# wenxiaoshuai/Points-Matching

Hardware: AMD Instinct MI355X
Metric: descriptor-pair distances/s (BF-L2 2-NN + ratio stage); RANSAC hypotheses/s in `ransac` (higher is better)
Workload: dtype f32

## Files before the change

points_matching_amd/csrc/knn_coarse_kernels.hpp:

```cpp
#pragma once
#include <type_traits>

#include "knn_shared.hpp"

namespace pm_knn {
namespace {

template <bool NO_EPI, bool NO_STAGE, bool NO_BARRIER, bool NO_LDSREAD>
struct Abl {
    static constexpr bool no_epi = NO_EPI;
    static constexpr bool no_stage = NO_STAGE;
    static constexpr bool no_barrier = NO_BARRIER;
    static constexpr bool no_ldsread = NO_LDSREAD;
    static __device__ __forceinline__ void stamp(int) {}
};
typedef Abl<false, false, false, false> AblNone;

struct WgTile { int qb, split; };
__device__ __forceinline__ WgTile wg_tile(bool tiled)
{
    const int nx = gridDim.x, ny = gridDim.y;
    if (!tiled || (nx & 3) || (ny & 1)) return WgTile{static_cast<int>(blockIdx.x), static_cast<int>(blockIdx.y)};
    const int L = blockIdx.y * nx + blockIdx.x;
    const int x = L & 7, j = L >> 3;
    const int tw = nx >> 2, th = ny >> 1;
    return WgTile{(x & 3) * tw + j % tw, (x >> 2) * th + j / tw};
}

template <typename ABL>
__device__ __forceinline__ void tile_barrier()
{
    if constexpr (ABL::no_barrier) asm volatile("" ::: "memory");
    else __syncthreads();
}

__device__ __forceinline__ float embed_lid(float w, unsigned keep_mask, unsigned lid)
{
    return __uint_as_float((__float_as_uint(w) & keep_mask) | (lid & ~keep_mask));
}

__device__ __forceinline__ void top4_insert(f32x4& c, float x)
{
    const float n0 = fmaxf(x, c[0]);
    const float n1 = __builtin_amdgcn_fmed3f(x, c[0], c[1]);
    const float n2 = __builtin_amdgcn_fmed3f(x, c[1], c[2]);
    const float n3 = __builtin_amdgcn_fmed3f(x, c[2], c[3]);
    c[0] = n0; c[1] = n1; c[2] = n2; c[3] = n3;
}

__device__ __forceinline__ void merge_halves(f32x4& cl, int h)
{
    f32x4 own, other;
#pragma unroll
    for (int i = 0; i < 4; ++i) {
        own[i] = __uint_as_float(__float_as_uint(cl[i]) | static_cast<unsigned>(h));
        other[i] = __shfl_xor(own[i], 32, 64);
    }
    cl = own;
#pragma unroll
    for (int i = 0; i < 4; ++i) top4_insert(cl, other[i]);
}

__device__ __forceinline__ float group_max(const f32x16& acc, int g)
{
    return fmaxf(fmaxf(fmaxf(acc[4 * g], acc[4 * g + 1]), acc[4 * g + 2]), acc[4 * g + 3]);
}

template <int NCH, bool FULL, int TT>
struct KnnTile {
    static constexpr int DP = NCH * 8;
    static constexpr int LDT = DP + 4;
    static constexpr int F4_PER_ROW = DP / 4;
    static constexpr int NSTG = TT * F4_PER_ROW / 256;
    static_assert(TT * F4_PER_ROW % 256 == 0, "tile must split evenly over the workgroup");

    f32x4 stg[NSTG];
    float stg_n;

    __device__ __forceinline__ void load(const float* __restrict__ T, const float* __restrict__ tnorm, int tile,
                                         int nt, int dim, int tid)
    {
#pragma unroll
        for (int i = 0; i < NSTG; ++i) {
            const int f = tid + 256 * i;
            const int row = f / F4_PER_ROW, c4 = f % F4_PER_ROW;
            int g = tile * TT + row;
            g = g < nt ? g : nt - 1;
            int col = 4 * c4;
            if (!FULL) col = col < dim ? col : dim - 4;
            f32x4 v = *reinterpret_cast<const f32x4*>(T + static_cast<size_t>(g) * dim + col);
            if (!FULL && 4 * c4 >= dim) v = f32x4{0.f, 0.f, 0.f, 0.f};
            stg[i] = v;
        }
        const int gn = tile * TT + (tid & (TT - 1));
        const float nrm = tnorm[gn < nt ? gn : nt - 1];
        stg_n = gn < nt ? -0.5f * nrm : -0.5f * KNN_BIG;
    }
    __device__ __forceinline__ void store(float* __restrict__ Ts, int buf, int tid) const
    {
#pragma unroll
        for (int i = 0; i < NSTG; ++i) {
            const int f = tid + 256 * i;
            const int row = f / F4_PER_ROW, c4 = f % F4_PER_ROW;
            *reinterpret_cast<f32x4*>(Ts + (buf * TT + row) * LDT + 4 * c4) = stg[i];
        }
        if (tid < TT) *reinterpret_cast<f32x4*>(Ts + (buf * TT + tid) * LDT + DP) = f32x4{stg_n, 0.f, 0.f, 0.f};
    }
};

template <int NCH, bool FULL, int NB, bool EPI, typename ABL>
__device__ __forceinline__ void knn_tile_compute(float* __restrict__ Ts, int buf, int r, int h,
                                                 const f32x4 (&qf)[NCH], f32x16 (&a)[NB], const f32x16 (&p)[NB],
                                                 unsigned pbase, unsigned keep_mask, f32x4& cl,
                                                 KnnTile<NCH, FULL, NB * 32>& st, const float* __restrict__ T,
                                                 const float* __restrict__ tnorm, int next_tile, int nt, int dim,
                                                 int tid)
{
    constexpr int DP = NCH * 8;
    constexpr int LDT = DP + 4;
    constexpr int TT = NB * 32;
    static_assert(NCH >= 4, "the in-chain schedule needs at least 4 chunks");
    const float* tb = Ts + buf * TT * LDT + r * LDT + 4 * h;
    const float one_or_zero = h == 0 ? 1.f : 0.f;
    float sda[NB];
    f32x4 xn[NB];
#pragma unroll
    for (int blk = 0; blk < NB; ++blk) {
        sda[blk] = Ts[buf * TT * LDT + (32 * blk + r) * LDT + DP + h];
        xn[blk] = *reinterpret_cast<const f32x4*>(tb + 32 * blk * LDT);
    }
    {
        const f32x16 zero = {0.f, 0.f, 0.f, 0.f, 0.f, 0.f, 0.f, 0.f, 0.f, 0.f, 0.f, 0.f, 0.f, 0.f, 0.f, 0.f};
#pragma unroll
        for (int blk = 0; blk < NB; ++blk)
            a[blk] = __builtin_amdgcn_mfma_f32_32x32x2f32(sda[blk], one_or_zero, zero, 0, 0, 0);
    }
#pragma unroll
    for (int c = 0; c < NCH; ++c) {
        f32x4 x[NB];
#pragma unroll
        for (int blk = 0; blk < NB; ++blk) x[blk] = xn[blk];
        if constexpr (!ABL::no_ldsread) {
            if (c + 1 < NCH) {
#pragma unroll
                for (int blk = 0; blk < NB; ++blk)
                    xn[blk] = *reinterpret_cast<const f32x4*>(tb + 32 * blk * LDT + 8 * (c + 1));
            }
        }
#pragma unroll
        for (int t = 0; t < 4; ++t)
#pragma unroll
            for (int blk = 0; blk < NB; ++blk)
                a[blk] = __builtin_amdgcn_mfma_f32_32x32x2f32(x[blk][t], qf[c][t], a[blk], 0, 0, 0);
        if constexpr (!ABL::no_stage) {
            if (c == 0) st.load(T, tnorm, next_tile, nt, dim, tid);
            if (c == NCH - 2) st.store(Ts, buf ^ 1, tid);
        }
        if (EPI && !ABL::no_epi) {
            constexpr int NG = 4 * NB;
#pragma unroll
            for (int g = (c == 0 ? 0 : (c - 1) * NG / (NCH - 1)); g < (c == 0 ? 0 : c * NG / (NCH - 1)); ++g)
                top4_insert(cl, embed_lid(group_max(p[g >> 2], g & 3), keep_mask, (pbase + static_cast<unsigned>(g)) << 1));
            asm volatile("" : "+v"(cl[0]), "+v"(cl[1]), "+v"(cl[2]), "+v"(cl[3]));
        }
    }
}

template <int NB>
__device__ __forceinline__ void knn_select_all(const f32x16 (&p)[NB], unsigned pbase, unsigned keep_mask, f32x4& cl)
{
#pragma unroll
    for (int g = 0; g < 4 * NB; ++g)
        top4_insert(cl, embed_lid(group_max(p[g >> 2], g & 3), keep_mask, (pbase + static_cast<unsigned>(g)) << 1));
}

template <int NCH, bool FULL, int TT, typename ABL>
__global__ __launch_bounds__(256, (TT == 64 ? 2 : 1)) void knn_l2_mfma(
    const float* __restrict__ Q, const float* __restrict__ T, const float* __restrict__ tnorm, int nq,
    int nt, int dim, int tiles_per_split, unsigned keep_mask, float* __restrict__ cand_val, int slots,
    const unsigned long long* __restrict__ stats, unsigned epoch, int only_if_ineligible)
{
    if (only_if_ineligible & 1) {
        const unsigned long long s1 = stats[1], s3 = stats[3];
        if (!(static_cast<unsigned>(s1 >> 32) == epoch && (s1 & 2ull) && static_cast<unsigned>(s3 >> 32) == epoch)) return;
    }
    using Tile = KnnTile<NCH, FULL, TT>;
    constexpr int LDT = Tile::LDT;
    constexpr int NB = TT / 32;
    constexpr unsigned IDS = 4 * NB;
    extern __shared__ __attribute__((aligned(16))) float smem[];
    float* Ts = smem;

    const int tid = threadIdx.x;
    const int lane = tid & 63, wave = tid >> 6;
    const int r = lane & 31, h = lane >> 5;
    const WgTile wg = wg_tile((only_if_ineligible & 2) != 0);
    const int qrow = wg.qb * QB + wave * 32 + r;
    const int qld = qrow < nq ? qrow : nq - 1;

    f32x4 qf[NCH];
#pragma unroll
    for (int c = 0; c < NCH; ++c) {
        const int k0 = 8 * c + 4 * h;
        int col = k0;
        if (!FULL) col = col < dim ? col : dim - 4;
        f32x4 v = *reinterpret_cast<const f32x4*>(Q + static_cast<size_t>(qld) * dim + col);
        if (!FULL && k0 >= dim) v = f32x4{0.f, 0.f, 0.f, 0.f};
        qf[c] = v;
    }

    const int ntiles = (nt + TT - 1) / TT;
    const int tile0 = wg.split * tiles_per_split;
    int tile1 = tile0 + tiles_per_split;
    if (tile1 > ntiles) tile1 = ntiles;

    f32x4 cl = {-KNN_BIG, -KNN_BIG, -KNN_BIG, -KNN_BIG};
    if (tile0 < tile1) {
        Tile st;
        st.load(T, tnorm, tile0, nt, dim, tid);
        st.store(Ts, 0, tid);
        __syncthreads();

        f32x16 accA[NB], accB[NB];
        int tix = 0;
        const int ntl = tile1 - tile0;
        knn_tile_compute<NCH, FULL, NB, false, ABL>(Ts, 0, r, h, qf, accA, accA, 0u, keep_mask, cl, st, T, tnorm,
                                               tile0 + 1, nt, dim, tid);
        tile_barrier<ABL>();
        ++tix;
        for (;;) {
            if (tix >= ntl) { knn_select_all<NB>(accA, static_cast<unsigned>(tix - 1) * IDS, keep_mask, cl); break; }
            knn_tile_compute<NCH, FULL, NB, true, ABL>(Ts, tix & 1, r, h, qf, accB, accA, static_cast<unsigned>(tix - 1) * IDS,
                                                  keep_mask, cl, st, T, tnorm, tile0 + tix + 1, nt, dim, tid);
            tile_barrier<ABL>();
            ++tix;
            if (tix >= ntl) { knn_select_all<NB>(accB, static_cast<unsigned>(tix - 1) * IDS, keep_mask, cl); break; }
            knn_tile_compute<NCH, FULL, NB, true, ABL>(Ts, tix & 1, r, h, qf, accA, accB, static_cast<unsigned>(tix - 1) * IDS,
                                                  keep_mask, cl, st, T, tnorm, tile0 + tix + 1, nt, dim, tid);
            tile_barrier<ABL>();
            ++tix;
        }
    }

    merge_halves(cl, h);
    if (qrow < nq && h == 0) {
        const size_t o = static_cast<size_t>(qrow) * slots + wg.split * KNN_C;
        *reinterpret_cast<f32x4*>(cand_val + o) = cl;
    }
}

template <int DP>
struct RouteF16T {
    static constexpr int NCH = DP / 16 + 1;
    static constexpr int ROW16 = (DP + 16) / 8;
    static constexpr int LDS_ROW16 = ROW16 + 1;
    static_assert(LDS_ROW16 % 2 == 1 && (H_TT * LDS_ROW16) % 64 == 0, "conflict-free rows, whole DMA pieces");
    static constexpr int GPB = 4;
    static constexpr bool MERGE = true;
    static constexpr bool SEEDED = false;
    typedef f16x8 frag;
    typedef f32x16 acc;
    typedef f32x4 list;
    static __device__ __forceinline__ acc zero()
    {
        return acc{0.f, 0.f, 0.f, 0.f, 0.f, 0.f, 0.f, 0.f, 0.f, 0.f, 0.f, 0.f, 0.f, 0.f, 0.f, 0.f};
    }
    static __device__ __forceinline__ acc mfma(frag a, frag b, acc c)
    {
        return __builtin_amdgcn_mfma_f32_32x32x16_f16(a, b, c, 0, 0, 0);
    }
    static __device__ __forceinline__ list empty() { return list{-KNN_BIG, -KNN_BIG, -KNN_BIG, -KNN_BIG}; }
    static __device__ __forceinline__ void select(const acc& a, unsigned par, unsigned gid, list& cl, int g)
    {
        top4_insert(cl, embed_lid(group_max(a, g), par, gid));
    }
    static __device__ __forceinline__ void merge(list& cl, int h) { merge_halves(cl, h); }
    static __device__ __forceinline__ void put(list& cl, float x) { top4_insert(cl, x); }
};
typedef RouteF16T<128> RouteF16;
static_assert(RouteF16::NCH == H_NCH && RouteF16::ROW16 == H_ROW16 && RouteF16::LDS_ROW16 == H_LDS_ROW16, "knn_shared.hpp constants");

template <int BITS>
struct RouteI8T {
    static_assert(BITS == 256 || BITS == 512, "descriptor bits padded to 256 or 512");
    static constexpr int NCH = BITS / 32;
    static constexpr int ROW16 = BITS / 16;
    static constexpr int LDS_ROW16 = ROW16 + 1;
    static_assert(LDS_ROW16 % 2 == 1 && (H_TT * LDS_ROW16) % 64 == 0, "conflict-free rows, whole DMA pieces");
    static constexpr int GPB = 2;
    static constexpr bool MERGE = false;
    static constexpr bool SEEDED = false;
    typedef i32x4 frag;
    typedef i32x16 acc;
    typedef i32x4 list;
    static __device__ __forceinline__ acc zero() { return acc{0, 0, 0, 0, 0, 0, 0, 0, 0, 0, 0, 0, 0, 0, 0, 0}; }
    static __device__ __forceinline__ acc mfma(frag a, frag b, acc c)
    {
        return __builtin_amdgcn_mfma_i32_32x32x32_i8(a, b, c, 0, 0, 0);
    }
    static __device__ __forceinline__ list empty() { return list{I8_EMPTY, I8_EMPTY, I8_EMPTY, I8_EMPTY}; }
    static __device__ __forceinline__ int med3(int a, int b, int c) { return max(min(a, b), min(max(a, b), c)); }
    static __device__ __forceinline__ void select(const acc& a, unsigned par, unsigned gid, list& cl, int g)
    {
        const int m0 = max(max(a[8 * g], a[8 * g + 1]), a[8 * g + 2]);
        const int m1 = max(max(a[8 * g + 3], a[8 * g + 4]), a[8 * g + 5]);
        const int m = max(max(max(m0, m1), a[8 * g + 6]), a[8 * g + 7]);
        const int x = static_cast<int>((static_cast<unsigned>(m) << I8_SHIFT) | gid);
        (void)par;
        insert(cl, x);
    }
    static __device__ __forceinline__ void put(list& cl, int x) { insert(cl, x); }
    static __device__ __forceinline__ void insert(list& cl, int x)
    {
        const int n0 = max(x, cl[0]);
        const int n1 = med3(x, cl[0], cl[1]);
        const int n2 = med3(x, cl[1], cl[2]);
        const int n3 = med3(x, cl[2], cl[3]);
        cl[0] = n0; cl[1] = n1; cl[2] = n2; cl[3] = n3;
    }
    static __device__ __forceinline__ void merge(list& cl, int h)
    {
#pragma unroll
        for (int i = 0; i < 4; ++i) cl[i] = cl[i] == I8_EMPTY ? I8_EMPTY : (cl[i] | h);
    }
};
struct RouteI8 : RouteI8T<I8_BITS> {};
static_assert(RouteI8::NCH == I8_NCH && RouteI8::ROW16 == I8_ROW16 && RouteI8::LDS_ROW16 == I8_LDS_ROW16, "knn_shared.hpp constants");
typedef RouteI8T<I8W_BITS> RouteI8W;
static_assert(RouteI8W::NCH == I8W_NCH && RouteI8W::ROW16 == I8W_ROW16 && RouteI8W::LDS_ROW16 == 33, "knn_shared.hpp constants");
static_assert(sizeof(uint4) * 2 * H_TT * RouteI8W::LDS_ROW16 == 135168, "two 512-bit tile buffers: one workgroup per CU");

struct RouteF16S : RouteF16 {
    static constexpr int NCH = F16S_NCH;
    static constexpr int ROW16 = F16S_ROW16;
    static constexpr int LDS_ROW16 = F16S_LDS_ROW16;
    static constexpr bool SEEDED = true;
};

template <int GPB_>
struct RouteU8T {
    static constexpr int NCH = U8_NCH;
    static constexpr int ROW16 = U8_ROW16;
    static constexpr int LDS_ROW16 = U8_LDS_ROW16;
    static constexpr int GPB = GPB_;
    static constexpr int GROUP = 16 / GPB_;
    static constexpr bool MERGE = true;
    static constexpr bool SEEDED = true;
    typedef i32x4 frag;
    typedef i32x16 acc;
    typedef i32x4 list;
    static __device__ __forceinline__ acc zero() { return acc{0, 0, 0, 0, 0, 0, 0, 0, 0, 0, 0, 0, 0, 0, 0, 0}; }
    static __device__ __forceinline__ acc mfma(frag a, frag b, acc c)
    {
        return __builtin_amdgcn_mfma_i32_32x32x32_i8(a, b, c, 0, 0, 0);
    }
    static __device__ __forceinline__ list empty() { return list{I8_EMPTY, I8_EMPTY, I8_EMPTY, I8_EMPTY}; }
    static __device__ __forceinline__ int max3(int a, int b, int c) { return max(max(a, b), c); }
    static __device__ __forceinline__ void select(const acc& a, unsigned par, unsigned gid, list& cl, int g)
    {
        int m;
        if constexpr (GROUP == 4) {
            m = max(max3(a[4 * g], a[4 * g + 1], a[4 * g + 2]), a[4 * g + 3]);
        } else if constexpr (GROUP == 8) {
            const int m0 = max3(a[8 * g], a[8 * g + 1], a[8 * g + 2]);
            const int m1 = max3(m0, a[8 * g + 3], a[8 * g + 4]);
            m = max(max3(m1, a[8 * g + 5], a[8 * g + 6]), a[8 * g + 7]);
        } else {
            const int m0 = max3(a[0], a[1], a[2]), m1 = max3(a[3], a[4], a[5]), m2 = max3(a[6], a[7], a[8]);
            const int m3 = max3(a[9], a[10], a[11]), m4 = max3(a[12], a[13], a[14]);
            m = max(max3(m0, m1, m2), max3(m3, m4, a[15]));
        }
        (void)par;
        RouteI8::insert(cl, static_cast<int>((static_cast<unsigned>(m) << U8_SHIFT) | gid));
    }
    static __device__ __forceinline__ void put(list& cl, int x) { RouteI8::insert(cl, x); }
    static __device__ __forceinline__ void merge(list& cl, int h)
    {
        list own, other;
#pragma unroll
        for (int i = 0; i < 4; ++i) {
            own[i] = cl[i] == I8_EMPTY ? I8_EMPTY : (cl[i] | h);
            other[i] = __shfl_xor(own[i], 32, 64);
        }
        cl = own;
#pragma unroll
        for (int i = 0; i < 4; ++i) RouteI8::insert(cl, other[i]);
    }
};
typedef RouteU8T<4> RouteU8;

template <typename R, int THREADS>
struct HTile {
    static constexpr int TOTAL = H_TT * R::ROW16;
    static constexpr int PIECES = (TOTAL + THREADS - 1) / THREADS;
    static constexpr bool EVEN = TOTAL % THREADS == 0;
    uint4 stg[PIECES];
    __device__ __forceinline__ void load(const uint4* __restrict__ Th, int tile, int tid)
    {
#pragma unroll
        for (int i = 0; i < PIECES; ++i) {
            int f = tid + THREADS * i;
            if (!EVEN) f = f < TOTAL ? f : TOTAL - 1;
            stg[i] = Th[static_cast<size_t>(tile) * TOTAL + f];
        }
    }
    __device__ __forceinline__ void store(uint4* __restrict__ hsm, int buf, int tid) const
    {
#pragma unroll
        for (int i = 0; i < PIECES; ++i) {
            const int f = tid + THREADS * i;
            const int row = f / R::ROW16, c8 = f % R::ROW16;
            if (EVEN || f < TOTAL) hsm[(buf * H_TT + row) * R::LDS_ROW16 + c8] = stg[i];
        }
    }
};

template <typename R, int THREADS>
struct HTileDma {
    static constexpr int NW = THREADS / 64;
    static constexpr int SLOTS = H_TT * R::LDS_ROW16;
    static_assert(SLOTS % 64 == 0, "the padded tile must be a whole number of 1-KiB pieces");
    static constexpr int NPIECES = SLOTS / 64;
    static constexpr int PER_WAVE = (NPIECES + NW - 1) / NW;
    static constexpr int TOTAL = H_TT * R::ROW16;
    unsigned src[PER_WAVE];
    __device__ __forceinline__ void init(int lane, int wave)
    {
#pragma unroll
        for (int i = 0; i < PER_WAVE; ++i) {
            const int p = wave + NW * i;
            const int s = 64 * (p < NPIECES ? p : NPIECES - 1) + lane;
            const int row = s / R::LDS_ROW16, c = s % R::LDS_ROW16;
            src[i] = static_cast<unsigned>(row * R::ROW16 + (c < R::ROW16 ? c : R::ROW16 - 1));
        }
    }
    __device__ __forceinline__ void issue(__amdgpu_buffer_rsrc_t rsrc, int tile, uint4* __restrict__ hsm, int buf, int wave) const
    {
        typedef __attribute__((address_space(3))) void* lptr_t;
        const int soff = tile * (TOTAL * 16);
#pragma unroll
        for (int i = 0; i < PER_WAVE; ++i) {
            const int p = wave + NW * i;
            if (p < NPIECES) {
                uint4* l = hsm + buf * SLOTS + 64 * p;
                __builtin_amdgcn_raw_ptr_buffer_load_lds(rsrc, (lptr_t)l, 16, static_cast<int>(src[i]) * 16, soff, 0, 0);
            }
        }
    }
};

struct Seed64 { uint4 v[4]; };
template <typename R, int NQB, bool EPI, typename ABL>
__device__ __forceinline__ void h_block(const uint4* __restrict__ tb, const uint4* __restrict__ sb,
                                        const typename R::frag (&qf)[NQB][R::NCH],
                                        typename R::acc (&a)[NQB], const typename R::acc (&p)[NQB], unsigned pbase,
                                        unsigned par, typename R::list (&cl)[NQB])
{
    typedef typename R::frag frag;
    typename R::acc seed = R::zero();
    if constexpr (R::SEEDED) seed = __builtin_bit_cast(typename R::acc, Seed64{{sb[0], sb[1], sb[2], sb[3]}});
    frag ring[3];
#pragma unroll
    for (int c = 0; c < 3; ++c) ring[c] = *reinterpret_cast<const frag*>(tb + 2 * c);
#pragma unroll
    for (int c = 0; c < R::NCH; ++c) {
        const frag x = ring[c % 3];
        if constexpr (!ABL::no_ldsread) {
            if (c + 3 < R::NCH) ring[c % 3] = *reinterpret_cast<const frag*>(tb + 2 * (c + 3));
        }
#pragma unroll
        for (int qb = 0; qb < NQB; ++qb) a[qb] = R::mfma(x, qf[qb][c], c == 0 ? seed : a[qb]);
        if constexpr (ABL::no_epi) {
            if (EPI && c == 1) {
#pragma unroll
                for (int qb = 0; qb < NQB; ++qb)
#pragma unroll
                    for (int e = 0; e < 16; ++e) asm volatile("" ::"v"(p[qb][e]));
            }
        }
        if (EPI && c >= 1 && !ABL::no_epi) {
            constexpr int NGB = R::GPB * NQB;
#pragma unroll
            for (int e = (c - 1) * NGB / (R::NCH - 1); e < c * NGB / (R::NCH - 1); ++e)
                R::select(p[e % NQB], par, (pbase + static_cast<unsigned>(e / NQB)) << 1, cl[e % NQB], e / NQB);
            if (NQB == 2)
                asm volatile("" : "+v"(cl[0][0]), "+v"(cl[0][1]), "+v"(cl[0][2]), "+v"(cl[0][3]), "+v"(cl[NQB - 1][0]),
                             "+v"(cl[NQB - 1][1]), "+v"(cl[NQB - 1][2]), "+v"(cl[NQB - 1][3]));
            else
                asm volatile("" : "+v"(cl[0][0]), "+v"(cl[0][1]), "+v"(cl[0][2]), "+v"(cl[0][3]));
        }
    }
}

template <typename R, int NQB, bool FIRST, typename ABL>
__device__ __forceinline__ void h_tile(const uint4* __restrict__ tb, const uint4* __restrict__ sb,
                                       const typename R::frag (&qf)[NQB][R::NCH], typename R::acc (&A)[NQB],
                                       typename R::acc (&B)[NQB], unsigned lb, unsigned par, typename R::list (&cl)[NQB])
{
    typedef typename R::frag frag;
    typedef typename R::acc acc;
    constexpr int NCH = R::NCH, STEPS = 4 * NCH, PF = 3;
    constexpr unsigned G = R::GPB;
    auto a_ptr = [&](int step) { return reinterpret_cast<const frag*>(tb + (step / NCH) * 32 * R::LDS_ROW16 + 2 * (step % NCH)); };
    auto seed_of = [&](int blk) {
        if constexpr (R::SEEDED) {
            const uint4* p = sb + 8 * blk;
            return __builtin_bit_cast(acc, Seed64{{p[0], p[1], p[2], p[3]}});
        } else {
            return R::zero();
        }
    };
    frag ring[PF];
#pragma unroll
    for (int i = 0; i < PF; ++i) ring[i] = *a_ptr(i);
    acc seed = seed_of(0);
#pragma unroll
    for (int s_ = 0; s_ < STEPS; ++s_) {
        const int blk = s_ / NCH, c = s_ % NCH;
        const frag x = ring[s_ % PF];
        if constexpr (!ABL::no_ldsread) {
            if (s_ + PF < STEPS) ring[s_ % PF] = *a_ptr(s_ + PF);
        }
        acc(&cur)[NQB] = (blk & 1) ? B : A;
        const acc(&prev)[NQB] = (blk & 1) ? A : B;
#pragma unroll
        for (int qb = 0; qb < NQB; ++qb) cur[qb] = R::mfma(x, qf[qb][c], c == 0 ? seed : cur[qb]);
        if (c == 0 && blk < 3) seed = seed_of(blk + 1);
        const bool epi = !(FIRST && blk == 0);
        if constexpr (ABL::no_epi) {
            if (epi && c == 1) {
#pragma unroll
                for (int qb = 0; qb < NQB; ++qb)
#pragma unroll
                    for (int e = 0; e < 16; ++e) asm volatile("" ::"v"(prev[qb][e]));
            }
        }
        if (epi && c >= 1 && !ABL::no_epi) {
            constexpr int NGB = R::GPB * NQB;
            const unsigned pbase = lb + G * static_cast<unsigned>(blk) - G;
#pragma unroll
            for (int e = (c - 1) * NGB / (NCH - 1); e < c * NGB / (NCH - 1); ++e)
                R::select(prev[e % NQB], par, (pbase + static_cast<unsigned>(e / NQB)) << 1, cl[e % NQB], e / NQB);
            if (NQB == 2)
                asm volatile("" : "+v"(cl[0][0]), "+v"(cl[0][1]), "+v"(cl[0][2]), "+v"(cl[0][3]), "+v"(cl[NQB - 1][0]),
                             "+v"(cl[NQB - 1][1]), "+v"(cl[NQB - 1][2]), "+v"(cl[NQB - 1][3]));
            else
                asm volatile("" : "+v"(cl[0][0]), "+v"(cl[0][1]), "+v"(cl[0][2]), "+v"(cl[0][3]));
        }
    }
}

template <typename R, int NQB, bool DMA, int GR, int S, typename ABL>
__global__ __launch_bounds__(H_QB / (32 * NQB) * 64 * GR, (R::NCH > 9 ? (NQB == 2 ? 1 : 2) : (NQB == 2 ? 2 : 4))) void knn_mfma_rows288(
    const uint4* __restrict__ Qh, const uint4* __restrict__ Th, const uint4* __restrict__ seeds_g, int nq, int nt,
    int tiles_per_split, unsigned par, typename R::list* __restrict__ cand_val, int slots,
    const unsigned long long* __restrict__ stats, unsigned epoch, int mode)
{
    static_assert(S == 1 || ((S == 2 || S == 4) && GR == 1 && DMA && R::SEEDED), "super-tiles: the seeded LDS-DMA form, one row group");
    ABL::stamp(0);
    typedef typename R::frag frag;
    typedef typename R::acc acc;
    typedef typename R::list list;
    constexpr int WPG = H_QB / (32 * NQB);
    constexpr int THREADS = WPG * 64 * GR;
    static_assert(GR == 1 || (GR == 2 && NQB == 2 && R::MERGE), "row groups: the 64-query form of a merged-list route");
    if (mode & 1) {
        const unsigned long long s1 = stats[1], s3 = stats[3];
        if (static_cast<unsigned>(s1 >> 32) == epoch && (s1 & 2ull) && static_cast<unsigned>(s3 >> 32) == epoch)
            return;
    }
    extern __shared__ __attribute__((aligned(16))) uint4 hsm[];
    static_assert(!R::SEEDED || DMA, "the seeded routes stage by LDS-DMA only");
    constexpr int TILE_SLOTS = H_TT * R::LDS_ROW16;
    uint4* const ssm = hsm + 2 * S * TILE_SLOTS;
    const int tid = threadIdx.x, lane = tid & 63, wave = tid >> 6;
    const int r = lane & 31, h = lane >> 5;
    const int gw = wave % WPG, grp = wave / WPG;
    const WgTile wg = wg_tile((mode & 2) != 0);
    const int qbase = wg.qb * H_QB + gw * 32 * NQB;

    HTile<R, THREADS> st;
    HTileDma<R, THREADS> dma;
    const int ntiles = (nt + H_TT - 1) / H_TT;
    const int tile0 = wg.split * tiles_per_split;
    const __amdgpu_buffer_rsrc_t t_rsrc = __builtin_amdgcn_make_buffer_rsrc(
        const_cast<uint4*>(Th), 0, ntiles * (H_TT * R::ROW16 * 16), 0x00020000);
    const __amdgpu_buffer_rsrc_t s_rsrc = __builtin_amdgcn_make_buffer_rsrc(
        const_cast<uint4*>(R::SEEDED ? seeds_g : Th), 0, (ntiles + 1) * SEED_TILE_BYTES, 0x00020000);
    auto seed_issue = [&](int tile, int buf, int i) {
        typedef __attribute__((address_space(3))) void* lptr_t;
        if (R::SEEDED && wave == THREADS / 64 - 1 - i)
            __builtin_amdgcn_raw_ptr_buffer_load_lds(s_rsrc, (lptr_t)(ssm + 64 * buf), 16, lane * 16, tile * SEED_TILE_BYTES, 0, 0);
    };
    int tile1 = tile0 + tiles_per_split;
    if (tile1 > ntiles) tile1 = ntiles;
    const int ntl = tile1 - tile0;
    static_assert(S <= THREADS / 64, "one wave per seed piece of a super-tile");
    auto super_issue = [&](int u, int b) {
#pragma unroll
        for (int i = 0; i < S; ++i) {
            if constexpr (S == 1) {
                const int t = tile0 + u < ntiles ? tile0 + u : (tile0 + u - 1 < ntiles ? tile0 + u - 1 : ntiles - 1);
                dma.issue(t_rsrc, t, hsm, b, wave);
                seed_issue(t, b, 0);
            } else if (S * u + i < ntl) {
                dma.issue(t_rsrc, tile0 + S * u + i, hsm, b * S + i, wave);
                seed_issue(tile0 + S * u + i, b * S + i, i);
            }
        }
    };
    ABL::stamp(18);
    if (DMA) {
        dma.init(lane, wave);
        super_issue(0, 0);
        ABL::stamp(19);
    } else {
        st.load(Th, tile0 < ntiles ? tile0 : ntiles - 1, tid);
    }
    frag qf[NQB][R::NCH];
#pragma unroll
    for (int qb = 0; qb < NQB; ++qb)
#pragma unroll
        for (int c = 0; c < R::NCH; ++c) {
            if constexpr (R::SEEDED && R::NCH == U8_NCH)
                qf[qb][c] = *reinterpret_cast<const frag*>(Qh + (static_cast<size_t>((qbase >> 5) + qb) * R::NCH + c) * 64 + lane);
            else
                qf[qb][c] = *reinterpret_cast<const frag*>(Qh + static_cast<size_t>(qbase + 32 * qb + r) * R::ROW16 + 2 * c + h);
        }
    ABL::stamp(1);
#pragma unroll
    for (int qb = 0; qb < NQB; ++qb)
#pragma unroll
        for (int c = 0; c < R::NCH; ++c) {
            typedef unsigned u32x4 __attribute__((ext_vector_type(4)));
            u32x4 t = __builtin_bit_cast(u32x4, qf[qb][c]);
            asm volatile("" : "+v"(t));
            qf[qb][c] = __builtin_bit_cast(frag, t);
        }

    list cl[NQB];
#pragma unroll
    for (int qb = 0; qb < NQB; ++qb) cl[qb] = R::empty();

    if (tile0 < tile1) {
        if (!DMA) st.store(hsm, 0, tid);
        __syncthreads();
        ABL::stamp(2);
        acc A[NQB], B[NQB];
        for (int u = 0; u < (ntl + S - 1) / S; ++u) {
            const int buf = u & 1;
            constexpr unsigned G = R::GPB;
            if constexpr (!ABL::no_stage) {
                if (DMA) super_issue(u + 1, buf ^ 1);
                else st.load(Th, tile0 + u + 1 < ntiles ? tile0 + u + 1 : tile0 + u, tid);
            }
            if constexpr (GR == 1) {
#pragma unroll
                for (int i = 0; i < S; ++i) {
                    const int tix = S * u + i;
                    if (S > 1 && tix >= ntl) break;
                    const uint4* tb = hsm + ((buf * S + i) * H_TT + r) * R::LDS_ROW16 + h;
                    const uint4* sb = ssm + 64 * (buf * S + i) + 4 * h;
                    const unsigned lb = static_cast<unsigned>(tix) * (4u * G);
                    if (tix == 0) h_block<R, NQB, false, ABL>(tb, sb, qf, A, A, 0u, par, cl);
                    else h_block<R, NQB, true, ABL>(tb, sb, qf, A, B, lb - G, par, cl);
                    h_block<R, NQB, true, ABL>(tb + 32 * R::LDS_ROW16, sb + 8, qf, B, A, lb, par, cl);
                    h_block<R, NQB, true, ABL>(tb + 64 * R::LDS_ROW16, sb + 16, qf, A, B, lb + G, par, cl);
                    if constexpr (!ABL::no_stage) {
                        if (!DMA) st.store(hsm, buf ^ 1, tid);
                    }
                    h_block<R, NQB, true, ABL>(tb + 96 * R::LDS_ROW16, sb + 24, qf, B, A, lb + 2u * G, par, cl);
                }
            } else {
                const int tix = u;
                const uint4* tb = hsm + (buf * H_TT + r) * R::LDS_ROW16 + h;
                const uint4* sb = ssm + 64 * buf + 4 * h;
                const unsigned lb = static_cast<unsigned>(tix) * (4u * G);
                const uint4* tg = tb + grp * 64 * R::LDS_ROW16;
                const uint4* sg = sb + 16 * grp;
                const unsigned gb = lb + 2u * static_cast<unsigned>(grp) * G;
                if (tix == 0) h_block<R, NQB, false, ABL>(tg, sg, qf, A, A, 0u, par, cl);
                else h_block<R, NQB, true, ABL>(tg, sg, qf, A, B, gb - 3u * G, par, cl);
                if constexpr (!ABL::no_stage) {
                    if (!DMA) st.store(hsm, buf ^ 1, tid);
                }
                h_block<R, NQB, true, ABL>(tg + 32 * R::LDS_ROW16, sg + 8, qf, B, A, gb, par, cl);
            }
            tile_barrier<ABL>();
            if (u < 13) ABL::stamp(3 + u);
        }
        const unsigned lb = static_cast<unsigned>(tile1 - tile0 - 1) * (4u * R::GPB) +
                            (GR == 1 ? 3u : 2u * static_cast<unsigned>(grp) + 1u) * R::GPB;
#pragma unroll
        for (int qb = 0; qb < NQB; ++qb)
#pragma unroll
            for (int g = 0; g < R::GPB; ++g) R::select(B[qb], par, (lb + static_cast<unsigned>(g)) << 1, cl[qb], g);
    }
    ABL::stamp(16);
    if constexpr (GR == 2) {
        list* xs = reinterpret_cast<list*>(hsm);
#pragma unroll
        for (int qb = 0; qb < NQB; ++qb) {
            R::merge(cl[qb], h);
            if (grp == 1) xs[(gw * NQB + qb) * 64 + lane] = cl[qb];
        }
        __syncthreads();
        if (grp == 1) return;
#pragma unroll
        for (int qb = 0; qb < NQB; ++qb) {
            const list o = xs[(gw * NQB + qb) * 64 + lane];
#pragma unroll
            for (int i = 0; i < 4; ++i) R::put(cl[qb], o[i]);
            const int q = qbase + 32 * qb + r;
            if (q < nq && h == 0) cand_val[(static_cast<size_t>(q) * slots + wg.split * KNN_C) / KNN_C] = cl[qb];
        }
        return;
    }
#pragma unroll
    for (int qb = 0; qb < NQB; ++qb) {
        const int q = qbase + 32 * qb + r;
        R::merge(cl[qb], h);
        if (R::MERGE) {
            if (q < nq && h == 0) cand_val[(static_cast<size_t>(q) * slots + wg.split * KNN_C) / KNN_C] = cl[qb];
        } else {
            if (q < nq) cand_val[(static_cast<size_t>(q) * slots + (wg.split * 2 + h) * KNN_C) / KNN_C] = cl[qb];
        }
    }
    ABL::stamp(17);
}

template <int N>
__device__ __forceinline__ void wait_vmcnt_imm() { asm volatile("s_waitcnt vmcnt(%0)" ::"n"(N) : "memory"); }
template <int BASE>
__device__ __forceinline__ void wait_tiles(int ahead, bool plus)
{
    static_assert(7 * (BASE + 1) <= 63, "vmcnt is a 6-bit counter");
#define PM_W(A_) case A_: if (plus) wait_vmcnt_imm<A_ * (BASE + 1)>(); else wait_vmcnt_imm<A_ * BASE>(); break;
    switch (ahead) {
        PM_W(1) PM_W(2) PM_W(3) PM_W(4) PM_W(5) PM_W(6) PM_W(7)
        default: wait_vmcnt_imm<0>(); break;
    }
#undef PM_W
}

template <typename FRAG>
__device__ __forceinline__ FRAG untracked_load16(const void* p)
{
    typedef unsigned u32x4 __attribute__((ext_vector_type(4)));
    u32x4 v;
    asm volatile("global_load_dwordx4 %0, %1, off" : "=&v"(v) : "v"(p) : "memory");
    return __builtin_bit_cast(FRAG, v);
}
template <typename FRAG>
__device__ __forceinline__ void pin_after_wait(FRAG& f)
{
    typedef unsigned u32x4 __attribute__((ext_vector_type(4)));
    u32x4 t = __builtin_bit_cast(u32x4, f);
    asm volatile("" : "+v"(t)::"memory");
    f = __builtin_bit_cast(FRAG, t);
}

template <typename R, int NQB, int WAVES, int NBUF, bool SPLIT, typename ABL>
__global__ __launch_bounds__(WAVES * 64, WAVES / 4) void knn_mfma_ring(
    const uint4* __restrict__ Qh, const uint4* __restrict__ Th, const uint4* __restrict__ seeds_g, int nq, int nt,
    int tiles_per_split, unsigned par, typename R::list* __restrict__ cand_val, int slots, int mode, int pro)
{
    typedef typename R::frag frag;
    typedef typename R::acc acc;
    typedef typename R::list list;
    constexpr int THREADS = WAVES * 64;
    constexpr int QB_WG = WAVES * 32 * NQB;
    constexpr int TILE_SLOTS = H_TT * R::LDS_ROW16;
    typedef HTileDma<R, THREADS> Dma;
    static_assert(NBUF >= 3 && NBUF <= 8, "ring of three to eight buffers (wait_tiles covers up to 7 tiles in flight)");
    extern __shared__ __attribute__((aligned(16))) uint4 hsm[];
    uint4* const ssm = hsm + NBUF * TILE_SLOTS;
    int* const arrive = reinterpret_cast<int*>(ssm + NBUF * 64);
    int* const done = arrive + NBUF;
    const int tid = threadIdx.x, lane = tid & 63, wave = tid >> 6;
    const int r = lane & 31, h = lane >> 5;
    const WgTile wg = wg_tile((mode & 2) != 0);
    const int qbase = wg.qb * QB_WG + wave * 32 * NQB;
    ABL::stamp(0);
    if constexpr (SPLIT) {
        if (tid < 2 * NBUF) arrive[tid] = 0;
        asm volatile("s_waitcnt lgkmcnt(0)" ::: "memory");
        __builtin_amdgcn_s_barrier();
        asm volatile("" ::: "memory");
    }
    auto poll = [&](int* ctr, int target) {
        for (;;) {
            const int v = __builtin_amdgcn_readfirstlane(__hip_atomic_load(ctr, __ATOMIC_RELAXED, __HIP_MEMORY_SCOPE_WORKGROUP));
            if (v >= target) break;
            __builtin_amdgcn_s_sleep(1);
        }
        asm volatile("" ::: "memory");
    };
    auto bump = [&](int* ctr) {
        if (lane == 0) __hip_atomic_fetch_add(ctr, 1, __ATOMIC_RELAXED, __HIP_MEMORY_SCOPE_WORKGROUP);
    };

    const int ntiles = (nt + H_TT - 1) / H_TT;
    const int tile0 = wg.split * tiles_per_split;
    int tile1 = tile0 + tiles_per_split;
    if (tile1 > ntiles) tile1 = ntiles;
    const int ntl = tile1 - tile0;

    frag qf[NQB][R::NCH];
#pragma unroll
    for (int qb = 0; qb < NQB; ++qb)
#pragma unroll
        for (int c = 0; c < R::NCH; ++c)
            qf[qb][c] = untracked_load16<frag>(Qh + static_cast<size_t>(qbase + 32 * qb + r) * R::ROW16 + 2 * c + h);

    const __amdgpu_buffer_rsrc_t t_rsrc = __builtin_amdgcn_make_buffer_rsrc(
        const_cast<uint4*>(Th), 0, ntiles * (H_TT * R::ROW16 * 16), 0x00020000);
    const __amdgpu_buffer_rsrc_t s_rsrc = __builtin_amdgcn_make_buffer_rsrc(
        const_cast<uint4*>(R::SEEDED ? seeds_g : Th), 0, (ntiles + 1) * SEED_TILE_BYTES, 0x00020000);
    Dma dma;
    dma.init(lane, wave);
    constexpr int BASE = Dma::NPIECES / Dma::NW;
    const int own = (Dma::NPIECES - wave + Dma::NW - 1) / Dma::NW + ((R::SEEDED && wave == Dma::NW - 1) ? 1 : 0);
    const bool plus = __builtin_amdgcn_readfirstlane(own) != BASE;
    static_assert(Dma::NPIECES >= Dma::NW, "every wave issues at least one piece");
    auto request = [&](int t) {
        typedef __attribute__((address_space(3))) void* lptr_t;
        const int buf = t % NBUF;
        dma.issue(t_rsrc, tile0 + t, hsm, buf, wave);
        if (R::SEEDED && wave == Dma::NW - 1)
            __builtin_amdgcn_raw_ptr_buffer_load_lds(s_rsrc, (lptr_t)(ssm + 64 * buf), 16, lane * 16, (tile0 + t) * SEED_TILE_BYTES, 0, 0);
    };
    int next = 0;
    auto pump = [&](int done_below, int most) {
        for (int n = 0; n < most && next < ntl && next < done_below + NBUF; ++n) {
            if constexpr (SPLIT) {
                if (next >= NBUF) poll(&done[next % NBUF], WAVES * (next / NBUF));
            }
            request(next);
            ++next;
        }
    };
    pump(0, pro);
    if constexpr (SPLIT) {
        if (ntl > 0) {
            asm volatile("s_waitcnt vmcnt(0)" ::: "memory");
            bump(&arrive[0]);
        }
    }
    ABL::stamp(1);

    list cl[NQB];
#pragma unroll
    for (int qb = 0; qb < NQB; ++qb) cl[qb] = R::empty();

    if (ntl > 0) {
        acc A[NQB], B[NQB];
        constexpr unsigned G = R::GPB;
#pragma unroll 1
        for (int tix = 0; tix < ntl; ++tix) {
            if constexpr (SPLIT) {
                if constexpr (!ABL::no_barrier) poll(&arrive[tix % NBUF], WAVES * (tix / NBUF + 1));
                if constexpr (!ABL::no_stage) pump(tix, 2);
                if (tix + 1 < ntl) {
                    wait_tiles<BASE>(next - 2 - tix, plus);
                    bump(&arrive[(tix + 1) % NBUF]);
                }
            } else {
                if (tix == 0) asm volatile("s_waitcnt vmcnt(0)" ::: "memory");
                else wait_tiles<BASE>(next - 1 - tix, plus);
                if constexpr (!ABL::no_barrier) __builtin_amdgcn_s_barrier();
                asm volatile("" ::: "memory");
            }
#pragma unroll
            for (int qb = 0; qb < NQB; ++qb)
#pragma unroll
                for (int c = 0; c < R::NCH; ++c) pin_after_wait(qf[qb][c]);
            __builtin_amdgcn_sched_barrier(0);
            if constexpr (!SPLIT && !ABL::no_stage) pump(tix, 2);
            if (tix < 14) ABL::stamp(2 + tix);
            const int buf = tix % NBUF;
            const uint4* tb = hsm + (buf * H_TT + r) * R::LDS_ROW16 + h;
            const uint4* sb = ssm + 64 * buf + 4 * h;
            const unsigned lb = static_cast<unsigned>(tix) * (4u * G);
            if (tix == 0) h_tile<R, NQB, true, ABL>(tb, sb, qf, A, B, lb, par, cl);
            else h_tile<R, NQB, false, ABL>(tb, sb, qf, A, B, lb, par, cl);
            if constexpr (SPLIT) {
                if (tix + NBUF < ntl) bump(&done[tix % NBUF]);
            }
        }
        const unsigned lb = static_cast<unsigned>(ntl - 1) * (4u * G) + 3u * G;
#pragma unroll
        for (int qb = 0; qb < NQB; ++qb)
#pragma unroll
            for (int g = 0; g < R::GPB; ++g) R::select(B[qb], par, (lb + static_cast<unsigned>(g)) << 1, cl[qb], g);
    }
    ABL::stamp(16);
#pragma unroll
    for (int qb = 0; qb < NQB; ++qb) {
        const int q = qbase + 32 * qb + r;
        R::merge(cl[qb], h);
        if (R::MERGE) {
            if (q < nq && h == 0) cand_val[(static_cast<size_t>(q) * slots + wg.split * KNN_C) / KNN_C] = cl[qb];
        } else {
            if (q < nq) cand_val[(static_cast<size_t>(q) * slots + (wg.split * 2 + h) * KNN_C) / KNN_C] = cl[qb];
        }
    }
    ABL::stamp(17);
}

template <typename R>
inline bool rows288_dma_ok(int nt) { return (static_cast<long long>(nt) + H_TT) * (R::ROW16 * 16) < 0x7FFFFFFFLL; }

inline bool xcd_tiled(const pm_ctx* ctx) { return ctx->opts[PM_OPT_KNN_XCD_TILE] != 1; }

template <int NCH, bool FULL, int TT, typename ABL>
int launch_mfma(pm_ctx* ctx, const float* dq, int nq, const float* dt, int nt, int dim, const float* tnorm, int splits,
                int tiles_per_split, unsigned keep_mask, float* cval, int slots, const unsigned long long* stats,
                unsigned epoch, int only_if_ineligible)
{
    constexpr int LDT = NCH * 8 + 4;
    const size_t lds = 2 * TT * LDT * sizeof(float);
    static bool attr_done_dev[PM_MAX_DEVICES] = {};
    bool& attr_done = attr_done_dev[ctx->device];
    if (!attr_done) {
        PM_HIP_CHECK(hipFuncSetAttribute(reinterpret_cast<const void*>(&knn_l2_mfma<NCH, FULL, TT, ABL>),
                                         hipFuncAttributeMaxDynamicSharedMemorySize, static_cast<int>(lds)));
        attr_done = true;
    }
    dim3 grid((nq + QB - 1) / QB, splits);
    const int mode = (only_if_ineligible ? 1 : 0) | (xcd_tiled(ctx) ? 2 : 0);
    pm::ScopedKernelTime t(ctx, "knn_l2_mfma");
    hipLaunchKernelGGL((knn_l2_mfma<NCH, FULL, TT, ABL>), grid, dim3(256), lds, ctx->stream, dq, dt, tnorm, nq, nt, dim,
                       tiles_per_split, keep_mask, cval, slots, stats, epoch, mode);
    PM_HIP_CHECK(hipGetLastError());
    return PM_OK;
}

template <typename ABL>
int coarse_f32_dispatch(pm_ctx* ctx, const float* dq, int nq, const float* dt, int nt, int dim, const float* tnorm,
                      int splits, int tiles_per_split, unsigned keep_mask, float* cval, int slots,
                      const unsigned long long* stats, unsigned epoch, int only_if_ineligible)
{
#define PM_LAUNCH_MFMA(NCH_, FULL_)                                                                              \
    launch_mfma<NCH_, FULL_, TT32, ABL>(ctx, dq, nq, dt, nt, dim, tnorm, splits, tiles_per_split, keep_mask, cval, slots, \
                                   stats, epoch, only_if_ineligible)
    if (dim == 128) return PM_LAUNCH_MFMA(16, true);
    if (dim == 64) return PM_LAUNCH_MFMA(8, true);
    if (dim == 32) return PM_LAUNCH_MFMA(4, true);
    if (dim < 32) return PM_LAUNCH_MFMA(4, false);
    if (dim < 64) return PM_LAUNCH_MFMA(8, false);
    return PM_LAUNCH_MFMA(16, false);
#undef PM_LAUNCH_MFMA
}

template <typename R, typename ABL>
int launch_rows288(pm_ctx* ctx, const char* name, const void* Qh, const void* Th, const void* seeds, int nq, int nq_pad, int nt,
                   int splits, int tiles_per_split, unsigned par, void* cval, int slots, const unsigned long long* stats,
                   unsigned epoch, int mode, int st = 1)
{
    constexpr bool SUPER = std::is_same<R, RouteU8T<2>>::value;
    PM_REQUIRE(st == 1 || (SUPER && (st == 2 || st == 4)), PM_E_INVALID, "super-tiles exist for the u8 route's 8-row groups only");
    auto lds_of = [](int s_) { return sizeof(uint4) * s_ * (2 * H_TT * R::LDS_ROW16 + (R::SEEDED ? 2 * 64 : 0)); };
    static_assert(!SUPER || 4 * sizeof(uint4) * (2 * H_TT * R::LDS_ROW16 + 2 * 64) <= 160 * 1024, "S = 4 exceeds the CU's LDS");
    const int nqb_opt = ctx->opts[PM_OPT_KNN_F16_WAVES];
    const int nqb = nqb_opt ? nqb_opt : (tiles_per_split <= 8 ? 1 : 2);
    if (nqb == 3) st = 1;
    const size_t lds = lds_of(st);
    if constexpr (SUPER) {
        if (st == 2) name = "knn_l2_mfma_u8_s2";
        if (st == 4) name = "knn_l2_mfma_u8_s4";
    }
    static bool attr_done_dev[PM_MAX_DEVICES] = {};
    bool& attr_done = attr_done_dev[ctx->device];
    if (!attr_done) {
#define PM_ATTR_S(NQB_, DMA_, GR_, S_)                                                                            \
    PM_HIP_CHECK(hipFuncSetAttribute(reinterpret_cast<const void*>(&knn_mfma_rows288<R, NQB_, DMA_, GR_, S_, ABL>),    \
                                     hipFuncAttributeMaxDynamicSharedMemorySize, static_cast<int>(lds_of(S_))))
#define PM_ATTR(NQB_, DMA_, GR_) PM_ATTR_S(NQB_, DMA_, GR_, 1)
        PM_ATTR(1, true, 1); PM_ATTR(2, true, 1);
        if constexpr (SUPER) { PM_ATTR_S(1, true, 1, 2); PM_ATTR_S(2, true, 1, 2); PM_ATTR_S(1, true, 1, 4); PM_ATTR_S(2, true, 1, 4); }
        if constexpr (!R::SEEDED) { PM_ATTR(1, false, 1); PM_ATTR(2, false, 1); }
        if constexpr (R::MERGE) {
            PM_ATTR(2, true, 2);
            if constexpr (!R::SEEDED) PM_ATTR(2, false, 2);
        }
// ... 426 lines not shown
```

Baseline: 2348 billion.

## Interleave next-tile DMA pieces between MFMA chunks of the first block

Splits the prefetch of the next descriptor tile into per-piece LDS DMA issues and interleaves them between the MFMA chunks of the first h_block, fencing each group with sched_barrier. The aim is to spread the load issue across compute instead of emitting a burst at loop start, so memory issue overlaps with matrix work. For the U8 route the old placement is kept; leftover partial pieces and seeds are still issued up front. It adds template machinery and scheduling constraints that could hurt instruction scheduling or register use.

```diff
diff --git a/points_matching_amd/csrc/knn_coarse_kernels.hpp b/points_matching_amd/csrc/knn_coarse_kernels.hpp
--- a/points_matching_amd/csrc/knn_coarse_kernels.hpp
+++ b/points_matching_amd/csrc/knn_coarse_kernels.hpp
@@ -12,6 +12,7 @@
     static constexpr bool no_stage = NO_STAGE;
     static constexpr bool no_barrier = NO_BARRIER;
     static constexpr bool no_ldsread = NO_LDSREAD;
+    static constexpr int dma_place = -1;
     static __device__ __forceinline__ void stamp(int) {}
 };
 typedef Abl<false, false, false, false> AblNone;
@@ -422,6 +423,7 @@
     static_assert(SLOTS % 64 == 0, "the padded tile must be a whole number of 1-KiB pieces");
     static constexpr int NPIECES = SLOTS / 64;
     static constexpr int PER_WAVE = (NPIECES + NW - 1) / NW;
+    static constexpr int FULL = NPIECES / NW;
     static constexpr int TOTAL = H_TT * R::ROW16;
     unsigned src[PER_WAVE];
     __device__ __forceinline__ void init(int lane, int wave)
@@ -434,27 +436,50 @@
             src[i] = static_cast<unsigned>(row * R::ROW16 + (c < R::ROW16 ? c : R::ROW16 - 1));
         }
     }
-    __device__ __forceinline__ void issue(__amdgpu_buffer_rsrc_t rsrc, int tile, uint4* __restrict__ hsm, int buf, int wave) const
+    __device__ __forceinline__ void issue_piece(__amdgpu_buffer_rsrc_t rsrc, int tile, uint4* __restrict__ hsm, int buf, int wave, int i) const
     {
         typedef __attribute__((address_space(3))) void* lptr_t;
         const int soff = tile * (TOTAL * 16);
-#pragma unroll
-        for (int i = 0; i < PER_WAVE; ++i) {
-            const int p = wave + NW * i;
-            if (p < NPIECES) {
-                uint4* l = hsm + buf * SLOTS + 64 * p;
-                __builtin_amdgcn_raw_ptr_buffer_load_lds(rsrc, (lptr_t)l, 16, static_cast<int>(src[i]) * 16, soff, 0, 0);
-            }
-        }
+        const int p = wave + NW * i;
+        if (i < FULL || p < NPIECES) {
+            uint4* l = hsm + buf * SLOTS + 64 * p;
+            __builtin_amdgcn_raw_ptr_buffer_load_lds(rsrc, (lptr_t)l, 16, static_cast<int>(src[i]) * 16, soff, 0, 0);
+        }
+    }
+    __device__ __forceinline__ void issue(__amdgpu_buffer_rsrc_t rsrc, int tile, uint4* __restrict__ hsm, int buf, int wave) const
+    {
+#pragma unroll
+        for (int i = 0; i < PER_WAVE; ++i) issue_piece(rsrc, tile, hsm, buf, wave, i);
     }
 };
 
+template <typename R>
+struct DmaPlace {
+    static constexpr int value = 1;
+};
+template <int GPB_>
+struct DmaPlace<RouteU8T<GPB_>> {
+    static constexpr int value = 0;
+};
+struct NoPieces {
+    static constexpr int N = 0;
+    __device__ __forceinline__ void operator()(int) const {}
+};
+template <int N_, typename F>
+struct Pieces {
+    static constexpr int N = N_;
+    F f;
+    __device__ __forceinline__ void operator()(int k) const { f(k); }
+};
+template <int N_, typename F>
+__device__ __forceinline__ Pieces<N_, F> make_pieces(F f) { return Pieces<N_, F>{f}; }
+
 struct Seed64 { uint4 v[4]; };
-template <typename R, int NQB, bool EPI, typename ABL>
+template <typename R, int NQB, bool EPI, typename ABL, typename PIECES = NoPieces>
 __device__ __forceinline__ void h_block(const uint4* __restrict__ tb, const uint4* __restrict__ sb,
                                         const typename R::frag (&qf)[NQB][R::NCH],
                                         typename R::acc (&a)[NQB], const typename R::acc (&p)[NQB], unsigned pbase,
-                                        unsigned par, typename R::list (&cl)[NQB])
+                                        unsigned par, typename R::list (&cl)[NQB], const PIECES& pieces = PIECES())
 {
     typedef typename R::frag frag;
     typename R::acc seed = R::zero();
@@ -470,6 +495,14 @@
         }
 #pragma unroll
         for (int qb = 0; qb < NQB; ++qb) a[qb] = R::mfma(x, qf[qb][c], c == 0 ? seed : a[qb]);
+        if constexpr (PIECES::N > 0) {
+            constexpr int FREE = 0x2 | 0x4 | 0x80 | 0x100 | 0x200;
+            __builtin_amdgcn_sched_barrier(FREE);
+            constexpr int PPC = (PIECES::N + R::NCH - 1) / R::NCH;
+#pragma unroll
+            for (int k = c * PPC; k < (c + 1) * PPC && k < PIECES::N; ++k) pieces(k);
+            __builtin_amdgcn_sched_barrier(FREE);
+        }
         if constexpr (ABL::no_epi) {
             if (EPI && c == 1) {
 #pragma unroll
@@ -600,14 +633,25 @@
 #pragma unroll
         for (int i = 0; i < S; ++i) {
             if constexpr (S == 1) {
-                const int t = tile0 + u < ntiles ? tile0 + u : (tile0 + u - 1 < ntiles ? tile0 + u - 1 : ntiles - 1);
-                dma.issue(t_rsrc, t, hsm, b, wave);
-                seed_issue(t, b, 0);
+                if (u == 0 || u < ntl) {
+                    const int t = tile0 + u < ntiles ? tile0 + u : (tile0 + u - 1 < ntiles ? tile0 + u - 1 : ntiles - 1);
+                    dma.issue(t_rsrc, t, hsm, b, wave);
+                    seed_issue(t, b, 0);
+                }
             } else if (S * u + i < ntl) {
                 dma.issue(t_rsrc, tile0 + S * u + i, hsm, b * S + i, wave);
                 seed_issue(tile0 + S * u + i, b * S + i, i);
             }
         }
+    };
+    constexpr int PLACE = !DMA || ABL::no_stage ? 0 : (ABL::dma_place >= 0 ? ABL::dma_place : DmaPlace<R>::value);
+    constexpr int NPC = PLACE != 0 ? HTileDma<R, THREADS>::FULL : 0;
+    const int wv = __builtin_amdgcn_readfirstlane(wave);
+    auto next_piece = [&](int nx, int b, int k) { dma.issue_piece(t_rsrc, tile0 + nx, hsm, b, wv, k); };
+    auto next_rest = [&](int nx, int b, int i) {
+        if constexpr (HTileDma<R, THREADS>::PER_WAVE > HTileDma<R, THREADS>::FULL)
+            dma.issue_piece(t_rsrc, tile0 + nx, hsm, b, wave, HTileDma<R, THREADS>::FULL);
+        seed_issue(tile0 + nx, b, i);
     };
     ABL::stamp(18);
     if (DMA) {
@@ -651,8 +695,13 @@
             const int buf = u & 1;
             constexpr unsigned G = R::GPB;
             if constexpr (!ABL::no_stage) {
-                if (DMA) super_issue(u + 1, buf ^ 1);
-                else st.load(Th, tile0 + u + 1 < ntiles ? tile0 + u + 1 : tile0 + u, tid);
+                if constexpr (!DMA) st.load(Th, tile0 + u + 1 < ntiles ? tile0 + u + 1 : tile0 + u, tid);
+                else if constexpr (PLACE == 0) super_issue(u + 1, buf ^ 1);
+                else {
+#pragma unroll
+                    for (int i = 0; i < S; ++i)
+                        if (S * (u + 1) + i < ntl) next_rest(S * (u + 1) + i, (buf ^ 1) * S + i, i);
+                }
             }
             if constexpr (GR == 1) {
 #pragma unroll
@@ -662,8 +711,13 @@
                     const uint4* tb = hsm + ((buf * S + i) * H_TT + r) * R::LDS_ROW16 + h;
                     const uint4* sb = ssm + 64 * (buf * S + i) + 4 * h;
                     const unsigned lb = static_cast<unsigned>(tix) * (4u * G);
-                    if (tix == 0) h_block<R, NQB, false, ABL>(tb, sb, qf, A, A, 0u, par, cl);
-                    else h_block<R, NQB, true, ABL>(tb, sb, qf, A, B, lb - G, par, cl);
+                    const int nx = tix + S;
+                    auto block0 = [&](const auto& pcs) {
+                        if (tix == 0) h_block<R, NQB, false, ABL>(tb, sb, qf, A, A, 0u, par, cl, pcs);
+                        else h_block<R, NQB, true, ABL>(tb, sb, qf, A, B, lb - G, par, cl, pcs);
+                    };
+                    if (NPC > 0 && nx < ntl) block0(make_pieces<NPC>([&](int k) { next_piece(nx, (buf ^ 1) * S + i, k); }));
+                    else block0(NoPieces());
                     h_block<R, NQB, true, ABL>(tb + 32 * R::LDS_ROW16, sb + 8, qf, B, A, lb, par, cl);
                     h_block<R, NQB, true, ABL>(tb + 64 * R::LDS_ROW16, sb + 16, qf, A, B, lb + G, par, cl);
                     if constexpr (!ABL::no_stage) {
@@ -679,8 +733,12 @@
                 const uint4* tg = tb + grp * 64 * R::LDS_ROW16;
                 const uint4* sg = sb + 16 * grp;
                 const unsigned gb = lb + 2u * static_cast<unsigned>(grp) * G;
-                if (tix == 0) h_block<R, NQB, false, ABL>(tg, sg, qf, A, A, 0u, par, cl);
-                else h_block<R, NQB, true, ABL>(tg, sg, qf, A, B, gb - 3u * G, par, cl);
+                auto block0 = [&](const auto& pcs) {
+                    if (tix == 0) h_block<R, NQB, false, ABL>(tg, sg, qf, A, A, 0u, par, cl, pcs);
+                    else h_block<R, NQB, true, ABL>(tg, sg, qf, A, B, gb - 3u * G, par, cl, pcs);
+                };
+                if (NPC > 0 && tix + 1 < ntl) block0(make_pieces<NPC>([&](int k) { next_piece(tix + 1, buf ^ 1, k); }));
+                else block0(NoPieces());
                 if constexpr (!ABL::no_stage) {
                     if (!DMA) st.store(hsm, buf ^ 1, tid);
                 }
```

After: 2307 billion. 1.8% lower.
